# yanqinJiang/Animate3D

Measured on NVIDIA H100. Metric: MV-VDM denoise-steps/sec @ 4view x 16frame x 256^2, higher is better.
Workload: dtype fp16

## Files before the change

### animate3d_b200/csrc/a3d_attn.cu

```cuda
#include <stdlib.h>

#include "a3d_common.cuh"
#include "a3d_host.cuh"
#include "a3d_wgmma.cuh"

namespace a3d {

struct AttnDev {
  int q_tiles, kv_tiles;
  int rows_q, rows_k;
  int heads;
  int q_t1, q_box1, q_box2, q_e1, q_e3;
  int k_t1, k_box1, k_box2, k_e3, kv_div, kv_i3_zero;
  uint32_t q_box_bytes, k_box_bytes;
  float scale_log2;
  __half* out;
  int64_t os1, os2, os3, os4;
  int accumulate;
  float out_scale;
  unsigned long long* dbg;
};

constexpr float kRescaleLog2 = 8.0f;
constexpr int kAttnThreads = 288;

template <int D>
struct AttnCfg {
  static constexpr int kDqk = (D + 15) / 16 * 16;
  static constexpr int kDv = (D + 1 + 15) / 16 * 16;
  static constexpr int kQB = (kDqk + 63) / 64;
  static constexpr int kVB = (kDv + 63) / 64;
  static constexpr int kStages = (D == 160) ? 3 : 4;
  static constexpr int kQBox = 128 * 128;
  static constexpr int kKVBox = 64 * 128;
  static constexpr int kSmemQ = kQB * kQBox;
  static constexpr int kSmemK = kStages * kQB * kKVBox;
  static constexpr int kSmemV = kStages * kVB * kKVBox;
  static constexpr int kSmemBytes = kSmemQ + kSmemK + kSmemV + 1024 + 256;
  static constexpr int kMinBlocks = (kSmemBytes <= 113 * 1024) ? 2 : 1;
  static_assert(kSmemBytes <= 227 * 1024, "shared memory budget");
};

template <int N>
__device__ __forceinline__ void wgmma_pv(float (&o)[N / 2], const uint32_t (&a)[4], uint64_t bdesc, uint32_t acc) {
  if constexpr (N == 48) wgmma_rs_n48<1>(o, a, bdesc, acc);
  else if constexpr (N == 96) wgmma_rs_n96<1>(o, a, bdesc, acc);
  else wgmma_rs_n176<1>(o, a, bdesc, acc);
}

template <int D>
__global__ void __launch_bounds__(kAttnThreads, AttnCfg<D>::kMinBlocks)
attn_tc_kernel(const AttnDev p, const __grid_constant__ CUtensorMap mapQ, const __grid_constant__ CUtensorMap mapK,
               const __grid_constant__ CUtensorMap mapV) {
  using Cfg = AttnCfg<D>;
  constexpr int S = Cfg::kStages;
  extern __shared__ uint8_t smem_raw[];
  uint8_t* smem = reinterpret_cast<uint8_t*>((reinterpret_cast<uintptr_t>(smem_raw) + 1023) & ~uintptr_t(1023));
  uint8_t* sQ = smem;
  uint8_t* sK = sQ + Cfg::kSmemQ;
  uint8_t* sV = sK + Cfg::kSmemK;
  uint64_t* bars = reinterpret_cast<uint64_t*>(sV + Cfg::kSmemV);
  uint64_t* q_full = bars;
  uint64_t* k_full = bars + 1;
  uint64_t* v_full = k_full + S;
  uint64_t* kv_empty = v_full + S;

  const int warp = threadIdx.x >> 5;
  const int lane = threadIdx.x & 31;
  const int qt = blockIdx.x;
  const int head = blockIdx.y;
  const int qb = blockIdx.z;
  const int n = p.kv_tiles;
  const int rows_tile = p.k_box1 * p.k_box2;

  if (p.rows_q < 128 || rows_tile < 64) {
    uint4* z = reinterpret_cast<uint4*>(sQ);
    const int n16 = (Cfg::kSmemQ + Cfg::kSmemK + Cfg::kSmemV) / 16;
    for (int i = threadIdx.x; i < n16; i += blockDim.x) z[i] = make_uint4(0, 0, 0, 0);
    fence_proxy_async_smem();
  }
  if (warp == 8 && lane == 0) {
    tma_prefetch_desc(&mapQ);
    tma_prefetch_desc(&mapK);
    tma_prefetch_desc(&mapV);
    mbar_init(q_full, 1);
    for (int i = 0; i < S; ++i) {
      mbar_init(&k_full[i], 1);
      mbar_init(&v_full[i], 1);
      mbar_init(&kv_empty[i], 8);
    }
    mbar_fence_init();
  }
  __syncthreads();

  const int q_i1 = (qt % p.q_t1) * p.q_box1;
  const int q_i2 = (qt / p.q_t1) * p.q_box2;
  const int q_i3 = qb % p.q_e3;
  const int q_i4 = qb / p.q_e3;

  if (warp == 8) {
    if (lane == 0) {
      const int kb = qb / p.kv_div;
      const int k_i3 = p.kv_i3_zero ? 0 : (kb % p.k_e3);
      const int k_i4 = kb / p.k_e3;
      mbar_expect_tx(q_full, p.q_box_bytes * Cfg::kQB);
#pragma unroll
      for (int b = 0; b < Cfg::kQB; ++b)
        tma_load_5d(sQ + b * Cfg::kQBox, &mapQ, q_full, head * Cfg::kDqk + b * 64, q_i1, q_i2, q_i3, q_i4);
      for (int j = 0; j < n; ++j) {
        const int st = j % S;
        const int k_i1 = (j % p.k_t1) * p.k_box1, k_i2 = (j / p.k_t1) * p.k_box2;
        mbar_wait(&kv_empty[st], ((j / S) & 1) ^ 1);
        mbar_expect_tx(&k_full[st], p.k_box_bytes * Cfg::kQB);
#pragma unroll
        for (int b = 0; b < Cfg::kQB; ++b)
          tma_load_5d(sK + (st * Cfg::kQB + b) * Cfg::kKVBox, &mapK, &k_full[st], head * Cfg::kDqk + b * 64, k_i1, k_i2, k_i3,
                      k_i4);
        mbar_expect_tx(&v_full[st], p.k_box_bytes * Cfg::kVB);
#pragma unroll
        for (int b = 0; b < Cfg::kVB; ++b)
          tma_load_5d(sV + (st * Cfg::kVB + b) * Cfg::kKVBox, &mapV, &v_full[st], head * Cfg::kDv + b * 64, k_i1, k_i2, k_i3,
                      k_i4);
      }
    }
    return;
  }

  const int wg = warp >> 2;
  const int g = lane >> 2, t = lane & 3;
  float s[32];
  float o[Cfg::kDv / 2];
#pragma unroll
  for (int i = 0; i < Cfg::kDv / 2; ++i) o[i] = 0.f;
  float m_lo = -INFINITY, m_hi = -INFINITY;
  const uint32_t q0 = smem_u32(sQ + wg * (64 * 128));
  mbar_wait(q_full, 0);
  for (int j = 0; j < n; ++j) {
    const int st = j % S;
    const uint32_t ph = (j / S) & 1;
    mbar_wait(&k_full[st], ph);
    wgmma_fence();
#pragma unroll
    for (int kk = 0; kk < Cfg::kDqk / 16; ++kk) {
      const uint64_t qd = make_smem_desc_sw128(q0 + (kk / 4) * Cfg::kQBox + (kk % 4) * 32, 16, 1024);
      const uint64_t kd = make_smem_desc_sw128(smem_u32(sK + (st * Cfg::kQB + kk / 4) * Cfg::kKVBox) + (kk % 4) * 32, 16, 1024);
      wgmma_ss_n64<0>(s, qd, kd, kk ? 1u : 0u);
    }
    wgmma_commit();
    wgmma_wait<0>();
    reg_fence(s);
    const int valid = (j == n - 1) ? p.rows_k : rows_tile;
    float mx_lo = -INFINITY, mx_hi = -INFINITY;
#pragma unroll
    for (int jj = 0; jj < 8; ++jj) {
#pragma unroll
      for (int e = 0; e < 2; ++e) {
        if (8 * jj + 2 * t + e >= valid) { s[4 * jj + e] = -INFINITY; s[4 * jj + 2 + e] = -INFINITY; }
        mx_lo = fmaxf(mx_lo, s[4 * jj + e]);
        mx_hi = fmaxf(mx_hi, s[4 * jj + 2 + e]);
      }
    }
#pragma unroll
    for (int x = 1; x <= 2; x <<= 1) {
      mx_lo = fmaxf(mx_lo, __shfl_xor_sync(0xffffffffu, mx_lo, x));
      mx_hi = fmaxf(mx_hi, __shfl_xor_sync(0xffffffffu, mx_hi, x));
    }
    const float mn_lo = fmaxf(m_lo, mx_lo * p.scale_log2), mn_hi = fmaxf(m_hi, mx_hi * p.scale_log2);
    if (j == 0) {
      m_lo = mn_lo; m_hi = mn_hi;
    } else if (__any_sync(0xffffffffu, mn_lo - m_lo > kRescaleLog2 || mn_hi - m_hi > kRescaleLog2)) {
      if (p.dbg && lane == 0) atomicAdd(p.dbg, 1ull);
      const float a_lo = ex2_approx(m_lo - mn_lo), a_hi = ex2_approx(m_hi - mn_hi);
#pragma unroll
      for (int c = 0; c < Cfg::kDv / 8; ++c) {
        o[4 * c] *= a_lo; o[4 * c + 1] *= a_lo; o[4 * c + 2] *= a_hi; o[4 * c + 3] *= a_hi;
      }
      m_lo = mn_lo; m_hi = mn_hi;
    }
    uint32_t pa[4][4];
#pragma unroll
    for (int kk = 0; kk < 4; ++kk) {
#pragma unroll
      for (int h = 0; h < 2; ++h) {
        const float* sb = s + 4 * (2 * kk + h);
        pa[kk][2 * h] = pack_f16x2(ex2_approx(fmaf(sb[0], p.scale_log2, -m_lo)), ex2_approx(fmaf(sb[1], p.scale_log2, -m_lo)));
        pa[kk][2 * h + 1] = pack_f16x2(ex2_approx(fmaf(sb[2], p.scale_log2, -m_hi)), ex2_approx(fmaf(sb[3], p.scale_log2, -m_hi)));
      }
    }
    mbar_wait(&v_full[st], ph);
    wgmma_fence();
#pragma unroll
    for (int kk = 0; kk < 4; ++kk) {
      const uint64_t vd = make_smem_desc_sw128(smem_u32(sV + st * Cfg::kVB * Cfg::kKVBox) + kk * 2048, Cfg::kKVBox, 1024);
      wgmma_pv<Cfg::kDv>(o, pa[kk], vd, 1u);
    }
    wgmma_commit();
    wgmma_wait<0>();
    reg_fence(o);
    __syncwarp();
    if (lane == 0) mbar_arrive(&kv_empty[st]);
  }
  const float l_lo = __shfl_sync(0xffffffffu, o[4 * (D / 8)], lane & ~3);
  const float l_hi = __shfl_sync(0xffffffffu, o[4 * (D / 8) + 2], lane & ~3);
#pragma unroll
  for (int h = 0; h < 2; ++h) {
    const int r = wg * 64 + (warp & 3) * 16 + g + 8 * h;
    const int i1 = q_i1 + r % p.q_box1;
    if (r >= p.rows_q || i1 >= p.q_e1) continue;
    const float inv = p.out_scale / (h ? l_hi : l_lo);
    const int i2 = q_i2 + r / p.q_box1;
    __half* orow = p.out + (int64_t)i1 * p.os1 + (int64_t)i2 * p.os2 + (int64_t)q_i3 * p.os3 + (int64_t)q_i4 * p.os4 +
                   head * D + 2 * t;
#pragma unroll
    for (int c = 0; c < D / 8; ++c) {
      float v0 = o[4 * c + 2 * h] * inv, v1 = o[4 * c + 2 * h + 1] * inv;
      if (p.accumulate) {
        const float2 f = __half22float2(*reinterpret_cast<const __half2*>(orow + 8 * c));
        v0 += f.x; v1 += f.y;
      }
      *reinterpret_cast<uint32_t*>(orow + 8 * c) = pack_f16x2(v0, v1);
    }
  }
}

struct ViewDev {
  const __half* base;
  int64_t s1, s2, s3, s4;
  int e1, e2, e3, e4;
};

__global__ void attn_simt_kernel(ViewDev q, ViewDev k, ViewDev v, __half* out, int64_t os1, int64_t os2, int64_t os3,
                                 int64_t os4, int heads, int d, int dqk, int dv, float scale, int kv_div, int kv_i3_zero,
                                 int accumulate, float out_scale) {
  const int Lq = q.e1 * q.e2, Lk = k.e1 * k.e2;
  const int64_t total = (int64_t)q.e3 * q.e4 * heads * Lq;
  const int64_t idx = (int64_t)blockIdx.x * blockDim.x + threadIdx.x;
  if (idx >= total) return;
  const int l = (int)(idx % Lq);
  const int h = (int)((idx / Lq) % heads);
  const int qb = (int)(idx / ((int64_t)Lq * heads));
  const int kb = qb / kv_div;
  const __half* qp = q.base + (int64_t)(l % q.e1) * q.s1 + (int64_t)(l / q.e1) * q.s2 + (int64_t)(qb % q.e3) * q.s3 +
                     (int64_t)(qb / q.e3) * q.s4 + h * dqk;
  const int64_t koff = (int64_t)(kv_i3_zero ? 0 : kb % k.e3) * k.s3 + (int64_t)(kb / k.e3) * k.s4;
  const int64_t voff = (int64_t)(kv_i3_zero ? 0 : kb % v.e3) * v.s3 + (int64_t)(kb / v.e3) * v.s4;
  float m = -INFINITY;
  for (int j = 0; j < Lk; ++j) {
    const __half* kp = k.base + koff + (int64_t)(j % k.e1) * k.s1 + (int64_t)(j / k.e1) * k.s2 + h * dqk;
    float s = 0.f;
    for (int c = 0; c < d; ++c) s += __half2float(qp[c]) * __half2float(kp[c]);
    m = fmaxf(m, s * scale);
  }
  float acc[160];
  for (int c = 0; c < d; ++c) acc[c] = 0.f;
  float sum = 0.f;
  for (int j = 0; j < Lk; ++j) {
    const __half* kp = k.base + koff + (int64_t)(j % k.e1) * k.s1 + (int64_t)(j / k.e1) * k.s2 + h * dqk;
    const __half* vp = v.base + voff + (int64_t)(j % v.e1) * v.s1 + (int64_t)(j / v.e1) * v.s2 + h * dv;
    float s = 0.f;
    for (int c = 0; c < d; ++c) s += __half2float(qp[c]) * __half2float(kp[c]);
    const float pj = expf(s * scale - m);
    sum += pj;
    for (int c = 0; c < d; ++c) acc[c] += pj * __half2float(vp[c]);
  }
  __half* op = out + (int64_t)(l % q.e1) * os1 + (int64_t)(l / q.e1) * os2 + (int64_t)(qb % q.e3) * os3 +
               (int64_t)(qb / q.e3) * os4 + h * d;
  for (int c = 0; c < d; ++c) {
    float o = out_scale * acc[c] / sum;
    if (accumulate) o += __half2float(op[c]);
    op[c] = __float2half_rn(o);
  }
}

constexpr int kFewKeysMax = 8;

template <int D>
__global__ void __launch_bounds__(256)
attn_fewkeys_kernel(ViewDev q, ViewDev k, ViewDev v, __half* out, int64_t os1, int64_t os2, int64_t os3, int64_t os4, int heads,
                    int dqk, int dv, float scale_log2, int kv_div, int kv_i3_zero, int accumulate, float out_scale) {
  constexpr int d = D;
  const int Lq = q.e1 * q.e2, Lk = k.e1 * k.e2;
  const int64_t total = (int64_t)q.e3 * q.e4 * Lq * heads;
  const int64_t idx = (int64_t)blockIdx.x * blockDim.x + threadIdx.x;
// ... 401 lines not shown
```

### animate3d_b200/csrc/a3d_gemm.cu

```cuda
#include <type_traits>

#include "a3d_common.cuh"
#include "a3d_host.cuh"
#include "a3d_wgmma.cuh"

namespace a3d {

struct GemmDev {
  int64_t M, N, K;
  int num_k_blocks;
  int tiles_m, tiles_n;
  int a_mode;
  int cpb;
  int conv_s;
  int tpi;
  int boh;
  int bimg;
  int tpr;
  int conv_pad;
  const float* bias;
  const float* rowbias;
  int64_t rb_ld, rb_div, rb_mod;
  float acc_scale;
  const __half* R1; int64_t ldr1; float r1_scale;
  const __half* R2; int64_t ldr2;
  void* C; int64_t ldc;
  int geglu, out_f32;
  int64_t perm_a, perm_b;
  long long* trace;
};

__device__ __forceinline__ float gelu_erf(float x) {
  float t;
  asm("rcp.approx.ftz.f32 %0, %1;" : "=f"(t) : "f"(fmaf(0.3275911f * 0.70710678118654752f, fabsf(x), 1.0f)));
  float poly = fmaf(1.061405429f, t, -1.453152027f);
  poly = fmaf(poly, t, 1.421413741f);
  poly = fmaf(poly, t, -0.284496736f);
  poly = fmaf(poly, t, 0.254829592f);
  const float xs = x * 0.84932180028801904f;
  const float e = ex2_approx(-xs * xs);
  const float erf_abs = fmaf(-(poly * t), e, 1.0f);
  const float h = 0.5f * x;
  return fmaf(fabsf(h), erf_abs, h);
}

__device__ __forceinline__ int64_t perm_row(int64_t m, int64_t a, int64_t b) {
  if (a == 0) return m;
  const int64_t ab = a * b;
  return (m / ab) * ab + (m % b) * a + (m / b) % a;
}

constexpr int kBM = 128;
constexpr int kBK = 64;
constexpr int kGemmThreads = 288;

template <int BN>
struct GemmCfg {
  static constexpr int kABytes = kBM * kBK * 2;
  static constexpr int kBBytes = BN * kBK * 2;
  static constexpr int kStageBytes = kABytes + kBBytes;
  static constexpr int kStages = (227 * 1024 - 1024 - 256) / kStageBytes > 6 ? 6 : (227 * 1024 - 1024 - 256) / kStageBytes;
  static constexpr int kSmemBytes = kStages * kStageBytes + 1024  + 256 ;
  static_assert(kSmemBytes <= 227 * 1024, "shared memory budget");
};

template <int BN>
__device__ __forceinline__ void wgmma_tile(float (&d)[BN / 2], uint64_t adesc, uint64_t bdesc, uint32_t acc) {
  if constexpr (BN == 256) wgmma_ss_n256<0>(d, adesc, bdesc, acc);
  else if constexpr (BN == 160) wgmma_ss_n160<0>(d, adesc, bdesc, acc);
  else wgmma_ss_n128<0>(d, adesc, bdesc, acc);
}

enum { kEpiPlain = 0, kEpiRes = 1, kEpiGeglu = 2, kEpiF32 = 3, kEpiGelu = 4 };

template <int BN, int EPI>
struct EpiChunk {
  static constexpr int G = BN == 256 ? 1 + (EPI == kEpiGeglu) : 2;
  static constexpr bool kAhead = BN != 256;
  float bias[G][2];
  float rb[2][G][2];
  uint32_t r1[2][G], r2[2][G];
};

template <int EPI, int G>
__device__ __forceinline__ constexpr int epi_group(int c, int s) {
  if constexpr (EPI != kEpiGeglu) {
    return c * G + s;
  } else {
    const int o = c * (G / 2) + s % (G / 2);
    return (o / 4) * 8 + o % 4 + (s >= G / 2 ? 4 : 0);
  }
}

__device__ __forceinline__ void prefetch_l2(const void* a) { asm volatile("prefetch.global.L2 [%0];" ::"l"(a)); }

template <int BN, int EPI>
__global__ void __launch_bounds__(kGemmThreads, 1)
gemm_tc_kernel(const GemmDev p, const __grid_constant__ CUtensorMap mapA, const __grid_constant__ CUtensorMap mapB) {
  static_assert(EPI != kEpiGeglu || BN % 64 == 0, "GEGLU pairs a value with its gate inside 64-column blocks");
  static_assert((BN / 8) % EpiChunk<BN, EPI>::G == 0, "the tile's column groups split into whole chunks");
  using Cfg = GemmCfg<BN>;
  constexpr int kStages = Cfg::kStages;
  extern __shared__ uint8_t smem_raw[];
  uint8_t* smem = reinterpret_cast<uint8_t*>((reinterpret_cast<uintptr_t>(smem_raw) + 1023) & ~uintptr_t(1023));
  uint8_t* smem_a = smem;
  uint8_t* smem_b = smem + kStages * Cfg::kABytes;
  uint64_t* full_bar = reinterpret_cast<uint64_t*>(smem + kStages * Cfg::kStageBytes);
  uint64_t* empty_bar = full_bar + kStages;

  const int warp = threadIdx.x >> 5;
  const int lane = threadIdx.x & 31;
  const int num_tiles = p.tiles_m * p.tiles_n;

  if (warp == 8 && lane == 0) {
    tma_prefetch_desc(&mapA);
    tma_prefetch_desc(&mapB);
    for (int i = 0; i < kStages; ++i) {
      mbar_init(&full_bar[i], 1);
      mbar_init(&empty_bar[i], 8);
    }
    mbar_fence_init();
  }
  __syncthreads();

  if (warp == 8) {
    if (lane == 0) {
      int stage = 0;
      uint32_t phase = 0;
      for (int tile = blockIdx.x; tile < num_tiles; tile += gridDim.x) {
        const int mt = tile / p.tiles_n, nt = tile % p.tiles_n;
        int img0 = 0, oh0 = 0, ow0 = 0;
        if (p.a_mode == A3D_A_CONV3) {
          if (p.tpr > 1) { img0 = mt / p.tpi; oh0 = (mt % p.tpi) / p.tpr; ow0 = ((mt % p.tpi) % p.tpr) * kBM; }
          else if (p.tpi > 0) { img0 = mt / p.tpi; oh0 = (mt % p.tpi) * p.boh; }
          else { img0 = mt * p.bimg; oh0 = 0; }
        }
        for (int kb = 0; kb < p.num_k_blocks; ++kb) {
          mbar_wait(&empty_bar[stage], phase ^ 1);
          mbar_expect_tx(&full_bar[stage], Cfg::kStageBytes);
          if (p.a_mode == A3D_A_CONV3) {
            const int tap = kb / p.cpb, c0 = (kb % p.cpb) * kBK;
            const int ky = tap / 3, kx = tap % 3;
            tma_load_5d(smem_a + stage * Cfg::kABytes, &mapA, &full_bar[stage], c0, ow0 * p.conv_s + kx - p.conv_pad,
                        oh0 * p.conv_s + ky - p.conv_pad, img0, 0);
          } else {
            tma_load_5d(smem_a + stage * Cfg::kABytes, &mapA, &full_bar[stage], kb * kBK, mt * kBM, 0, 0, 0);
          }
          tma_load_5d(smem_b + stage * Cfg::kBBytes, &mapB, &full_bar[stage], kb * kBK, nt * BN, 0, 0, 0);
          if (++stage == kStages) { stage = 0; phase ^= 1; }
        }
      }
    }
    return;
  }

  const int wg = warp >> 2;
  const int g = lane >> 2, t = lane & 3;
  int stage = 0;
  uint32_t phase = 0;
  int tcount = 0;
  float acc[BN / 2];
  for (int tile = blockIdx.x; tile < num_tiles; tile += gridDim.x, ++tcount) {
    const int mt = tile / p.tiles_n, nt = tile % p.tiles_n;
    const bool tr = p.trace && blockIdx.x == 0 && threadIdx.x == 0 && tcount < 60;
    if (tr) p.trace[tcount * 16 + 0] = clock64();
    const int64_t col_base = (int64_t)nt * BN + 2 * t;
    int64_t row[2], orow[2];
#pragma unroll
    for (int h = 0; h < 2; ++h) {
      row[h] = (int64_t)mt * kBM + wg * 64 + (warp & 3) * 16 + g + 8 * h;
      orow[h] = (EPI == kEpiRes) ? perm_row(row[h], p.perm_a, p.perm_b) : row[h];
    }
    int prev_stage = -1;
    for (int kb = 0; kb < p.num_k_blocks; ++kb) {
      if constexpr (EPI == kEpiRes) {
        if (kb == (p.num_k_blocks > 2 ? p.num_k_blocks - 2 : 0)) {
          const int64_t ncols = p.N - (int64_t)nt * BN < BN ? p.N - (int64_t)nt * BN : BN;
          auto fetch = [&](const __half* a, bool ok) {
            const uintptr_t e = reinterpret_cast<uintptr_t>(a + ncols), l0 = reinterpret_cast<uintptr_t>(a) & ~uintptr_t(127);
#pragma unroll
            for (int i = 0; i < (2 * BN / 128 + 4) / 4; ++i) {
              const uintptr_t l = l0 + 128 * (t + 4 * i);
              if (ok && l < e) prefetch_l2(reinterpret_cast<const void*>(l));
            }
          };
#pragma unroll
          for (int h = 0; h < 2; ++h) {
            fetch(p.R1 + row[h] * p.ldr1 + (int64_t)nt * BN, p.R1 && row[h] < p.M);
            fetch(p.R2 + orow[h] * p.ldr2 + (int64_t)nt * BN, p.R2 && row[h] < p.M);
          }
        }
      }
      mbar_wait(&full_bar[stage], phase);
      const uint32_t a0 = smem_u32(smem_a + stage * Cfg::kABytes + wg * (64 * 128));
      const uint32_t b0 = smem_u32(smem_b + stage * Cfg::kBBytes);
      wgmma_fence();
#pragma unroll
      for (int k = 0; k < kBK / 16; ++k)
        wgmma_tile<BN>(acc, make_smem_desc_sw128(a0 + 32 * k, 16, 1024), make_smem_desc_sw128(b0 + 32 * k, 16, 1024),
                       (kb | k) ? 1u : 0u);
      wgmma_commit();
      wgmma_wait<1>();
      if (prev_stage >= 0 && lane == 0) mbar_arrive(&empty_bar[prev_stage]);
      prev_stage = stage;
      if (++stage == kStages) { stage = 0; phase ^= 1; }
    }

    using Chunk = EpiChunk<BN, EPI>;
    constexpr int G = Chunk::G;
    constexpr int kChunks = BN / 8 / G;
    const float* rb[2];
#pragma unroll
    for (int h = 0; h < 2; ++h) rb[h] = p.rowbias ? p.rowbias + ((row[h] / p.rb_div) % p.rb_mod) * p.rb_ld : nullptr;
    Chunk op;
    auto load_chunk = [&](int c) {
#pragma unroll
      for (int s = 0; s < G; ++s) {
        const int64_t n = col_base + 8 * epi_group<EPI, G>(c, s);
        const bool col_ok = n < p.N;
        op.bias[s][0] = (p.bias && col_ok) ? p.bias[n] : 0.f;
        op.bias[s][1] = (p.bias && col_ok) ? p.bias[n + 1] : 0.f;
#pragma unroll
        for (int h = 0; h < 2; ++h) {
          const bool ok = col_ok && row[h] < p.M;
          op.rb[h][s][0] = (rb[h] && ok) ? rb[h][n] : 0.f;
          op.rb[h][s][1] = (rb[h] && ok) ? rb[h][n + 1] : 0.f;
          if constexpr (EPI == kEpiRes) {
            op.r1[h][s] = (p.R1 && ok) ? *reinterpret_cast<const uint32_t*>(p.R1 + row[h] * p.ldr1 + n) : 0u;
            op.r2[h][s] = (p.R2 && ok) ? *reinterpret_cast<const uint32_t*>(p.R2 + orow[h] * p.ldr2 + n) : 0u;
          }
        }
      }
    };
    auto finish = [&](float v, int h, int s, int e) {
      if (p.bias) v += op.bias[s][e];
      if (rb[h]) v += op.rb[h][s][e];
      return v * p.acc_scale;
    };
    auto half2_float2 = [](uint32_t u) { return __half22float2(*reinterpret_cast<const __half2*>(&u)); };

    if constexpr (Chunk::kAhead) load_chunk(0);
    wgmma_wait<0>();
    reg_fence(acc);
    if (lane == 0) mbar_arrive(&empty_bar[prev_stage]);
    if (tr) p.trace[tcount * 16 + 1] = clock64();

#pragma unroll
    for (int c = 0; c < kChunks; ++c) {
      if constexpr (!Chunk::kAhead) load_chunk(c);
      if constexpr (EPI == kEpiGeglu) {
        uint32_t out[2][G / 2];
#pragma unroll
        for (int h = 0; h < 2; ++h)
#pragma unroll
          for (int s = 0; s < G / 2; ++s) {
            const int ju = epi_group<EPI, G>(c, s), jg = epi_group<EPI, G>(c, s + G / 2);
            const float u0 = finish(acc[4 * ju + 2 * h], h, s, 0), u1 = finish(acc[4 * ju + 2 * h + 1], h, s, 1);
            const float g0 = finish(acc[4 * jg + 2 * h], h, s + G / 2, 0), g1 = finish(acc[4 * jg + 2 * h + 1], h, s + G / 2, 1);
            out[h][s] = pack_f16x2(u0 * gelu_erf(g0), u1 * gelu_erf(g1));
          }
        if (Chunk::kAhead && c + 1 < kChunks) load_chunk(c + 1);
#pragma unroll
        for (int h = 0; h < 2; ++h) {
          if (row[h] >= p.M) continue;
          __half* crow = reinterpret_cast<__half*>(p.C) + row[h] * p.ldc;
#pragma unroll
          for (int s = 0; s < G / 2; ++s) {
            if (col_base + 8 * epi_group<EPI, G>(c, s) >= p.N) continue;
            const int o = c * (G / 2) + s;
            *reinterpret_cast<uint32_t*>(crow + (int64_t)nt * (BN / 2) + 8 * o + 2 * t) = out[h][s];
          }
        }
      } else if constexpr (EPI == kEpiF32) {
        float out[2][G][2];
#pragma unroll
        for (int h = 0; h < 2; ++h)
#pragma unroll
          for (int s = 0; s < G; ++s)
#pragma unroll
            for (int e = 0; e < 2; ++e) out[h][s][e] = finish(acc[4 * (c * G + s) + 2 * h + e], h, s, e);
        if (Chunk::kAhead && c + 1 < kChunks) load_chunk(c + 1);
#pragma unroll
        for (int h = 0; h < 2; ++h) {
          if (row[h] >= p.M) continue;
          float* crow = reinterpret_cast<float*>(p.C) + row[h] * p.ldc;
#pragma unroll
          for (int s = 0; s < G; ++s) {
            const int64_t n = col_base + 8 * (c * G + s);
            if (n >= p.N) continue;
            crow[n] = out[h][s][0];
            crow[n + 1] = out[h][s][1];
// ... 11 lines not shown
              v0 = gelu_erf(v0); v1 = gelu_erf(v1);
            }
            if constexpr (EPI == kEpiRes) {
              if (p.R1) {
                const float2 f = half2_float2(op.r1[h][s]);
                v0 += p.r1_scale * f.x; v1 += p.r1_scale * f.y;
              }
              if (p.R2) {
                const float2 f = half2_float2(op.r2[h][s]);
                v0 += f.x; v1 += f.y;
              }
            }
            out[h][s] = pack_f16x2(v0, v1);
          }
        if (Chunk::kAhead && c + 1 < kChunks) load_chunk(c + 1);
#pragma unroll
        for (int h = 0; h < 2; ++h) {
          if (row[h] >= p.M) continue;
          __half* crow = reinterpret_cast<__half*>(p.C) + orow[h] * p.ldc;
#pragma unroll
          for (int s = 0; s < G; ++s) {
            const int64_t n = col_base + 8 * (c * G + s);
            if (n >= p.N) continue;
            *reinterpret_cast<uint32_t*>(crow + n) = out[h][s];
          }
        }
      }
    }
    if (tr) p.trace[tcount * 16 + 2] = clock64();
  }
}

struct SimtConv { int n, h, w, c, s, oh, ow, pad; };

__global__ void gemm_simt_kernel(const GemmDev p, const __half* __restrict__ A, int64_t lda, const __half* __restrict__ B,
                                 SimtConv cv) {
  const int64_t n_out = p.geglu == 1 ? p.N / 2 : p.N;
  const int64_t idx = (int64_t)blockIdx.x * blockDim.x + threadIdx.x;
  if (idx >= p.M * n_out) return;
  const int64_t m = idx / n_out;
  const int64_t j = idx % n_out;
  auto dot = [&](int64_t n) {
    float acc = 0.f;
    const __half* b = B + n * p.K;
    if (p.a_mode == A3D_A_PLAIN) {
      const __half* a = A + m * lda;
      for (int64_t k = 0; k < p.K; ++k) acc += __half2float(a[k]) * __half2float(b[k]);
    } else {
      const int img = (int)(m / (cv.oh * cv.ow));
      const int oy = (int)((m / cv.ow) % cv.oh), ox = (int)(m % cv.ow);
      for (int tap = 0; tap < 9; ++tap) {
        const int iy = oy * cv.s + tap / 3 - cv.pad, ix = ox * cv.s + tap % 3 - cv.pad;
        if (iy < 0 || iy >= cv.h || ix < 0 || ix >= cv.w) continue;
        const __half* a = A + (((int64_t)img * cv.h + iy) * cv.w + ix) * cv.c;
        const __half* bb = b + (int64_t)tap * cv.c;
        for (int c = 0; c < cv.c; ++c) acc += __half2float(a[c]) * __half2float(bb[c]);
      }
    }
    return acc;
  };
  const int64_t orow = perm_row(m, p.perm_a, p.perm_b);
  const float* rb = p.rowbias ? p.rowbias + ((m / p.rb_div) % p.rb_mod) * p.rb_ld : nullptr;
  auto finish = [&](int64_t n) {
    float v = dot(n);
    if (p.bias) v += p.bias[n];
    if (rb) v += rb[n];
    return v * p.acc_scale;
  };
  if (p.geglu == 1) {
    const int64_t blk = j / 32, e = j % 32;
    const int64_t nu = blk * 64 + e, ng = nu + 32;
    const float u = finish(nu), g = finish(ng);
    reinterpret_cast<__half*>(p.C)[orow * p.ldc + j] = __float2half_rn(u * gelu_erf(g));
    return;
  }
  float v = finish(j);
  if (p.geglu == 2) v = gelu_erf(v);
  if (p.R1) v += p.r1_scale * __half2float(p.R1[m * p.ldr1 + j]);
  if (p.R2) v += __half2float(p.R2[orow * p.ldr2 + j]);
  if (p.out_f32) reinterpret_cast<float*>(p.C)[orow * p.ldc + j] = v;
  else reinterpret_cast<__half*>(p.C)[orow * p.ldc + j] = __float2half_rn(v);
}

template <int BN, int EPI>
static int launch_tc_epi(const GemmDev& dev, const CUtensorMap* mapA, const CUtensorMap* mapB, cudaStream_t st) {
  using Cfg = GemmCfg<BN>;
  static bool attr_set = false;
  if (!attr_set) {
    A3D_CUDA_CHECK(cudaFuncSetAttribute(gemm_tc_kernel<BN, EPI>, cudaFuncAttributeMaxDynamicSharedMemorySize, Cfg::kSmemBytes));
    attr_set = true;
  }
  const int tiles = dev.tiles_m * dev.tiles_n;
  const int grid = tiles < sm_count() ? tiles : sm_count();
  gemm_tc_kernel<BN, EPI><<<grid, kGemmThreads, Cfg::kSmemBytes, st>>>(dev, *mapA, *mapB);
  A3D_LAUNCH_CHECK();
  return A3D_OK;
}

template <int BN>
static int launch_tc(const GemmDev& dev, const CUtensorMap* mapA, const CUtensorMap* mapB, cudaStream_t st) {
  if (dev.out_f32) return launch_tc_epi<BN, kEpiF32>(dev, mapA, mapB, st);
  if (dev.geglu == 1) {
    if constexpr (BN % 64 == 0) return launch_tc_epi<BN, kEpiGeglu>(dev, mapA, mapB, st);
    else return fail(A3D_EINVAL, "a3d_gemm: GEGLU needs a 128- or 256-column tile");
  }
  if (dev.geglu == 2) return launch_tc_epi<BN, kEpiGelu>(dev, mapA, mapB, st);
  if (dev.R1 || dev.R2 || dev.perm_a) return launch_tc_epi<BN, kEpiRes>(dev, mapA, mapB, st);
  return launch_tc_epi<BN, kEpiPlain>(dev, mapA, mapB, st);
}

static long long* g_gemm_trace = nullptr;

}

extern "C" int a3d_debug_set_gemm_trace(void* device_buffer_1024_int64) {
  a3d::g_gemm_trace = reinterpret_cast<long long*>(device_buffer_1024_int64);
  return A3D_OK;
}

extern "C" int a3d_gemm(const a3d_gemm_args* a, void* stream) {
  using namespace a3d;
  cudaStream_t st = reinterpret_cast<cudaStream_t>(stream);
  if (!a || !a->A || !a->B || !a->C) return fail(A3D_EINVAL, "a3d_gemm: null operand");
  if (a->M <= 0 || a->N <= 0 || a->K <= 0) return fail(A3D_EINVAL, "a3d_gemm: empty problem M=%lld N=%lld K=%lld",
                                                        (long long)a->M, (long long)a->N, (long long)a->K);
  GemmDev d;
  memset(&d, 0, sizeof(d));
  d.M = a->M; d.N = a->N; d.K = a->K;
  d.a_mode = a->a_mode;
  d.bias = a->bias; d.rowbias = a->rowbias; d.rb_ld = a->rb_ld;
  d.rb_div = a->rb_div > 0 ? a->rb_div : 1; d.rb_mod = a->rb_mod > 0 ? a->rb_mod : (int64_t)1 << 40;
  d.acc_scale = a->acc_scale;
  d.R1 = reinterpret_cast<const __half*>(a->R1); d.ldr1 = a->ldr1; d.r1_scale = a->r1_scale;
  d.R2 = reinterpret_cast<const __half*>(a->R2); d.ldr2 = a->ldr2;
  d.C = a->C; d.ldc = a->ldc; d.geglu = a->geglu; d.out_f32 = a->out_f32;
  d.perm_a = a->perm_a; d.perm_b = a->perm_b;
  d.trace = g_gemm_trace;
  if (a->geglu < 0 || a->geglu > 2) return fail(A3D_EINVAL, "a3d_gemm: geglu must be 0 (none), 1 (GEGLU) or 2 (GELU)");
  const bool geglu = a->geglu == 1;
  if (geglu && (a->out_f32 || a->R1 || a->R2 || a->perm_a || (a->N % 128)))
    return fail(A3D_EINVAL, "a3d_gemm: GEGLU epilogue takes bias / row-bias only, fp16 output, N %% 128 == 0");
  if (a->geglu == 2 && (a->out_f32 || a->R1 || a->R2 || a->perm_a))
    return fail(A3D_EINVAL, "a3d_gemm: GELU epilogue takes bias / row-bias only, fp16 output");
  if (a->out_f32 && (a->R1 || a->R2 || a->perm_a))
    return fail(A3D_EINVAL, "a3d_gemm: fp32 output supports bias / row-bias only");

  SimtConv cv{0, 0, 0, 0, 1, 0, 0};
  if (a->a_mode == A3D_A_CONV3) {
    const int s = a->conv_stride;
    if (s != 1 && s != 2) return fail(A3D_EINVAL, "a3d_gemm: conv stride must be 1 or 2");
    if (a->conv_h % s || a->conv_w % s) return fail(A3D_EINVAL, "a3d_gemm: conv H/W must be multiples of the stride");
    cv = SimtConv{a->conv_n, a->conv_h, a->conv_w, a->conv_c, s, a->conv_h / s, a->conv_w / s, a->conv_nopad_lo ? 0 : 1};
    if (a->K != 9LL * a->conv_c || a->M != (int64_t)cv.n * cv.oh * cv.ow)
      return fail(A3D_EINVAL, "a3d_gemm: conv geometry does not match M/K");
    d.conv_s = s;
  } else if (a->a_mode != A3D_A_PLAIN) {
    return fail(A3D_EINVAL, "a3d_gemm: unknown a_mode %d", a->a_mode);
  }

  bool tc_ok = (a->K % kBK == 0) && (a->N % (geglu ? 16 : 8) == 0) && ((reinterpret_cast<uintptr_t>(a->A) & 15) == 0) &&
               ((reinterpret_cast<uintptr_t>(a->B) & 15) == 0) && (a->ldc % 16 == 0) &&
               ((reinterpret_cast<uintptr_t>(a->C) & 31) == 0);
  if (a->a_mode == A3D_A_PLAIN) tc_ok = tc_ok && (a->lda % 8 == 0) && a->lda >= a->K;
  int boh = 0, bimg = 1, tpi = 0, tpr = 1;
  if (a->a_mode == A3D_A_CONV3) {
    tc_ok = tc_ok && (cv.c % kBK == 0);
    const int opix = cv.oh * cv.ow;
    if (cv.ow > kBM) {
      tc_ok = tc_ok && (cv.ow % kBM == 0);
      boh = 1; tpr = cv.ow / kBM; tpi = cv.oh * tpr; bimg = 1;
    } else if (opix >= kBM) {
      tc_ok = tc_ok && (opix % kBM == 0) && (kBM % cv.ow == 0);
      boh = kBM / cv.ow; tpi = opix / kBM; bimg = 1;
    } else {
      tc_ok = tc_ok && (kBM % opix == 0);
      boh = cv.oh; tpi = 0; bimg = kBM / (opix > 0 ? opix : 1);
    }
    tc_ok = tc_ok && (tpr > 1 ? kBM : cv.ow) * cv.s <= 256 && boh * cv.s <= 256;
  }
  if (a->R1) tc_ok = tc_ok && (a->ldr1 % 16 == 0) && ((reinterpret_cast<uintptr_t>(a->R1) & 31) == 0);
  if (a->R2) tc_ok = tc_ok && (a->ldr2 % 16 == 0) && ((reinterpret_cast<uintptr_t>(a->R2) & 31) == 0);
  int impl = a->impl;
  if (impl == A3D_GEMM_AUTO) impl = tc_ok ? A3D_GEMM_TCGEN05 : A3D_GEMM_SIMT;
  if (impl == A3D_GEMM_TCGEN05 && !tc_ok)
    return fail(A3D_EINVAL, "a3d_gemm: shape/alignment not supported by the tensor-core path (M=%lld N=%lld K=%lld)",
                (long long)a->M, (long long)a->N, (long long)a->K);

  if (impl == A3D_GEMM_SIMT) {
    const int64_t n_out = geglu ? a->N / 2 : a->N;
    const int64_t total = a->M * n_out;
    const int threads = 128;
    const int64_t blocks = (total + threads - 1) / threads;
    gemm_simt_kernel<<<(unsigned)blocks, threads, 0, st>>>(d, reinterpret_cast<const __half*>(a->A), a->lda,
                                                           reinterpret_cast<const __half*>(a->B), cv);
    A3D_LAUNCH_CHECK();
    return A3D_OK;
  }

  int BN;
  if (geglu) BN = (a->N % 256 == 0) ? 256 : 128;
  else if (a->N % 256 == 0) BN = 256;
  else if (a->K <= 640 && a->N > 512 && (256 * ((a->N + 255) / 256) - a->N) * 8 <= a->N) {
    BN = 256;
  } else if (a->N % 160 == 0) BN = 160;
  else BN = 128;
  {
    static int force = -1;
    if (force < 0) { const char* e = getenv("A3D_GEMM_BN"); force = e ? atoi(e) : 0; }
    if (!geglu && (force == 128 || force == 160 || force == 256)) BN = force;
  }
  if (geglu && a->N % BN) return fail(A3D_EINVAL, "a3d_gemm: GEGLU needs N %% 128 == 0");
  d.num_k_blocks = (int)(a->K / kBK);
  d.tiles_m = (int)((a->M + kBM - 1) / kBM);
  d.tiles_n = (int)((a->N + BN - 1) / BN);
  d.cpb = a->a_mode == A3D_A_CONV3 ? cv.c / kBK : 0;
  d.tpi = tpi; d.boh = boh; d.bimg = bimg; d.tpr = tpr; d.conv_pad = cv.pad;
  const CUtensorMap *mapA = nullptr, *mapB = nullptr;
  {
    MapKey kb;
    const uint64_t dims[5] = {(uint64_t)a->K, (uint64_t)a->N, 1, 1, 1};
    const uint64_t str[4] = {(uint64_t)a->K, (uint64_t)a->K * a->N, (uint64_t)a->K * a->N, (uint64_t)a->K * a->N};
    const uint32_t box[5] = {kBK, (uint32_t)BN, 1, 1, 1};
    kb = make_key(a->B, dims, str, box);
    if (int r = get_tensor_map(kb, &mapB)) return r;
  }
  if (a->a_mode == A3D_A_PLAIN) {
    const uint64_t dims[5] = {(uint64_t)a->K, (uint64_t)a->M, 1, 1, 1};
    const uint64_t str[4] = {(uint64_t)a->lda, (uint64_t)a->lda * a->M, (uint64_t)a->lda * a->M, (uint64_t)a->lda * a->M};
    const uint32_t box[5] = {kBK, kBM, 1, 1, 1};
    MapKey ka = make_key(a->A, dims, str, box);
    if (int r = get_tensor_map(ka, &mapA)) return r;
  } else {
    const uint64_t img = (uint64_t)cv.h * cv.w * cv.c;
    const uint64_t dims[5] = {(uint64_t)cv.c, (uint64_t)cv.w, (uint64_t)cv.h, (uint64_t)cv.n, 1};
    const uint64_t str[4] = {(uint64_t)cv.c, (uint64_t)cv.w * cv.c, img, img * cv.n};
    const uint32_t box[5] = {kBK, (uint32_t)((tpr > 1 ? kBM : cv.ow) * cv.s), (uint32_t)(boh * cv.s), (uint32_t)bimg, 1};
    MapKey ka = make_key(a->A, dims, str, box);
    ka.estr[1] = cv.s; ka.estr[2] = cv.s;
    if (int r = get_tensor_map(ka, &mapA)) return r;
  }
  switch (BN) {
    case 256: return launch_tc<256>(d, mapA, mapB, st);
    case 160: return launch_tc<160>(d, mapA, mapB, st);
    default: return launch_tc<128>(d, mapA, mapB, st);
  }
}
```

Measured before the change: 5.657.

## Overlap next QK^T wgmma with current PV wgmma in attention consumer loop

Restructures the consumer warpgroup loop so the S=QK^T wgmma for tile j is issued before the PV wgmma for tile j-1, then waits with wgmma_wait<1> so the softmax of tile j runs while PV is still in flight. The goal is to hide tensor-core latency behind exp/max work. For D=40 the old serial order is kept. It also precomputes the smem descriptors once, skips masking for full tiles, and replaces launch_bounds with a __maxnreg__ cap. The extra live registers (P fragments plus scores plus O) may cause spills, especially at large head dims.

```diff
diff --git a/animate3d_b200/csrc/a3d_attn.cu b/animate3d_b200/csrc/a3d_attn.cu
--- a/animate3d_b200/csrc/a3d_attn.cu
+++ b/animate3d_b200/csrc/a3d_attn.cu
@@ -38,6 +38,8 @@
   static constexpr int kSmemV = kStages * kVB * kKVBox;
   static constexpr int kSmemBytes = kSmemQ + kSmemK + kSmemV + 1024 + 256;
   static constexpr int kMinBlocks = (kSmemBytes <= 113 * 1024) ? 2 : 1;
+  static constexpr bool kPipelined = D != 40;
+  static constexpr int kMaxRegs = 65536 / (kMinBlocks * kAttnThreads) / 8 * 8;
   static_assert(kSmemBytes <= 227 * 1024, "shared memory budget");
 };
 
@@ -49,7 +51,7 @@
 }
 
 template <int D>
-__global__ void __launch_bounds__(kAttnThreads, AttnCfg<D>::kMinBlocks)
+__global__ void __maxnreg__(AttnCfg<D>::kMaxRegs)
 attn_tc_kernel(const AttnDev p, const __grid_constant__ CUtensorMap mapQ, const __grid_constant__ CUtensorMap mapK,
                const __grid_constant__ CUtensorMap mapV) {
   using Cfg = AttnCfg<D>;
@@ -128,34 +130,47 @@
 
   const int wg = warp >> 2;
   const int g = lane >> 2, t = lane & 3;
+  const float sl2 = p.scale_log2;
   float s[32];
   float o[Cfg::kDv / 2];
+  uint32_t pa[4][4];
 #pragma unroll
   for (int i = 0; i < Cfg::kDv / 2; ++i) o[i] = 0.f;
   float m_lo = -INFINITY, m_hi = -INFINITY;
-  const uint32_t q0 = smem_u32(sQ + wg * (64 * 128));
-  mbar_wait(q_full, 0);
-  for (int j = 0; j < n; ++j) {
-    const int st = j % S;
-    const uint32_t ph = (j / S) & 1;
-    mbar_wait(&k_full[st], ph);
+  const uint64_t qdesc = make_smem_desc_sw128(smem_u32(sQ + wg * (64 * 128)), 16, 1024);
+  const uint64_t kdesc = make_smem_desc_sw128(smem_u32(sK), 16, 1024);
+  const uint64_t vdesc = make_smem_desc_sw128(smem_u32(sV), Cfg::kKVBox, 1024);
+
+  auto issue_s = [&](int st) {
+    const uint64_t kst = kdesc + (uint32_t)(st * (Cfg::kQB * Cfg::kKVBox / 16));
     wgmma_fence();
 #pragma unroll
-    for (int kk = 0; kk < Cfg::kDqk / 16; ++kk) {
-      const uint64_t qd = make_smem_desc_sw128(q0 + (kk / 4) * Cfg::kQBox + (kk % 4) * 32, 16, 1024);
-      const uint64_t kd = make_smem_desc_sw128(smem_u32(sK + (st * Cfg::kQB + kk / 4) * Cfg::kKVBox) + (kk % 4) * 32, 16, 1024);
-      wgmma_ss_n64<0>(s, qd, kd, kk ? 1u : 0u);
-    }
+    for (int kk = 0; kk < Cfg::kDqk / 16; ++kk)
+      wgmma_ss_n64<0>(s, qdesc + ((kk / 4) * Cfg::kQBox + (kk % 4) * 32) / 16, kst + ((kk / 4) * Cfg::kKVBox + (kk % 4) * 32) / 16,
+                      kk ? 1u : 0u);
     wgmma_commit();
-    wgmma_wait<0>();
-    reg_fence(s);
-    const int valid = (j == n - 1) ? p.rows_k : rows_tile;
-    float mx_lo = -INFINITY, mx_hi = -INFINITY;
+  };
+  auto issue_pv = [&](int st) {
+    const uint64_t vst = vdesc + (uint32_t)(st * (Cfg::kVB * Cfg::kKVBox / 16));
+    wgmma_fence();
+#pragma unroll
+    for (int kk = 0; kk < 4; ++kk) wgmma_pv<Cfg::kDv>(o, pa[kk], vst + kk * 2048 / 16, 1u);
+    wgmma_commit();
+  };
+  auto row_max = [&](int valid, float& mx_lo, float& mx_hi) {
+    if (valid < 64) {
+#pragma unroll
+      for (int jj = 0; jj < 8; ++jj) {
+#pragma unroll
+        for (int e = 0; e < 2; ++e)
+          if (8 * jj + 2 * t + e >= valid) { s[4 * jj + e] = -INFINITY; s[4 * jj + 2 + e] = -INFINITY; }
+      }
+    }
+    mx_lo = -INFINITY; mx_hi = -INFINITY;
 #pragma unroll
     for (int jj = 0; jj < 8; ++jj) {
 #pragma unroll
       for (int e = 0; e < 2; ++e) {
-        if (8 * jj + 2 * t + e >= valid) { s[4 * jj + e] = -INFINITY; s[4 * jj + 2 + e] = -INFINITY; }
         mx_lo = fmaxf(mx_lo, s[4 * jj + e]);
         mx_hi = fmaxf(mx_hi, s[4 * jj + 2 + e]);
       }
@@ -165,40 +180,101 @@
       mx_lo = fmaxf(mx_lo, __shfl_xor_sync(0xffffffffu, mx_lo, x));
       mx_hi = fmaxf(mx_hi, __shfl_xor_sync(0xffffffffu, mx_hi, x));
     }
-    const float mn_lo = fmaxf(m_lo, mx_lo * p.scale_log2), mn_hi = fmaxf(m_hi, mx_hi * p.scale_log2);
-    if (j == 0) {
-      m_lo = mn_lo; m_hi = mn_hi;
-    } else if (__any_sync(0xffffffffu, mn_lo - m_lo > kRescaleLog2 || mn_hi - m_hi > kRescaleLog2)) {
-      if (p.dbg && lane == 0) atomicAdd(p.dbg, 1ull);
-      const float a_lo = ex2_approx(m_lo - mn_lo), a_hi = ex2_approx(m_hi - mn_hi);
-#pragma unroll
-      for (int c = 0; c < Cfg::kDv / 8; ++c) {
-        o[4 * c] *= a_lo; o[4 * c + 1] *= a_lo; o[4 * c + 2] *= a_hi; o[4 * c + 3] *= a_hi;
-      }
-      m_lo = mn_lo; m_hi = mn_hi;
-    }
-    uint32_t pa[4][4];
+  };
+  auto exp_scores = [&]() {
+#pragma unroll
+    for (int i = 0; i < 32; i += 4) {
+      s[i] = ex2_approx(fmaf(s[i], sl2, -m_lo)); s[i + 1] = ex2_approx(fmaf(s[i + 1], sl2, -m_lo));
+      s[i + 2] = ex2_approx(fmaf(s[i + 2], sl2, -m_hi)); s[i + 3] = ex2_approx(fmaf(s[i + 3], sl2, -m_hi));
+    }
+  };
+  auto pack_p = [&]() {
 #pragma unroll
     for (int kk = 0; kk < 4; ++kk) {
 #pragma unroll
       for (int h = 0; h < 2; ++h) {
         const float* sb = s + 4 * (2 * kk + h);
-        pa[kk][2 * h] = pack_f16x2(ex2_approx(fmaf(sb[0], p.scale_log2, -m_lo)), ex2_approx(fmaf(sb[1], p.scale_log2, -m_lo)));
-        pa[kk][2 * h + 1] = pack_f16x2(ex2_approx(fmaf(sb[2], p.scale_log2, -m_hi)), ex2_approx(fmaf(sb[3], p.scale_log2, -m_hi)));
-      }
-    }
-    mbar_wait(&v_full[st], ph);
-    wgmma_fence();
-#pragma unroll
-    for (int kk = 0; kk < 4; ++kk) {
-      const uint64_t vd = make_smem_desc_sw128(smem_u32(sV + st * Cfg::kVB * Cfg::kKVBox) + kk * 2048, Cfg::kKVBox, 1024);
-      wgmma_pv<Cfg::kDv>(o, pa[kk], vd, 1u);
-    }
-    wgmma_commit();
+        pa[kk][2 * h] = pack_f16x2(sb[0], sb[1]);
+        pa[kk][2 * h + 1] = pack_f16x2(sb[2], sb[3]);
+      }
+    }
+  };
+
+  mbar_wait(q_full, 0);
+  mbar_wait(&k_full[0], 0);
+  issue_s(0);
+  wgmma_wait<0>();
+  reg_fence(s);
+  {
+    float mx_lo, mx_hi;
+    row_max(n == 1 ? p.rows_k : rows_tile, mx_lo, mx_hi);
+    m_lo = fmaxf(m_lo, mx_lo * sl2); m_hi = fmaxf(m_hi, mx_hi * sl2);
+  }
+  exp_scores();
+  pack_p();
+  if constexpr (!Cfg::kPipelined) {
+    mbar_wait(&v_full[0], 0);
+    issue_pv(0);
     wgmma_wait<0>();
     reg_fence(o);
     __syncwarp();
-    if (lane == 0) mbar_arrive(&kv_empty[st]);
+    if (lane == 0) mbar_arrive(&kv_empty[0]);
+  }
+  int st = 0;
+  uint32_t ph = 0;
+  for (int j = 1; j < n; ++j) {
+    const int pst = st;
+    const uint32_t pph = ph;
+    if (++st == S) { st = 0; ph ^= 1; }
+    mbar_wait(&k_full[st], ph);
+    issue_s(st);
+    if constexpr (Cfg::kPipelined) {
+      mbar_wait(&v_full[pst], pph);
+      issue_pv(pst);
+      wgmma_wait<1>();
+    } else {
+      wgmma_wait<0>();
+    }
+    reg_fence(s);
+    float mx_lo, mx_hi;
+    row_max(j == n - 1 ? p.rows_k : rows_tile, mx_lo, mx_hi);
+    const float mn_lo = fmaxf(m_lo, mx_lo * sl2), mn_hi = fmaxf(m_hi, mx_hi * sl2);
+    const bool rescale = __any_sync(0xffffffffu, mn_lo - m_lo > kRescaleLog2 || mn_hi - m_hi > kRescaleLog2);
+    float a_lo = 1.f, a_hi = 1.f;
+    if (rescale) {
+      a_lo = ex2_approx(m_lo - mn_lo); a_hi = ex2_approx(m_hi - mn_hi);
+      m_lo = mn_lo; m_hi = mn_hi;
+    }
+    exp_scores();
+    if (rescale && p.dbg && lane == 0) atomicAdd(p.dbg, 1ull);
+    if constexpr (Cfg::kPipelined) {
+      reg_fence(s);
+      wgmma_wait<0>();
+      reg_fence(o);
+      __syncwarp();
+      if (lane == 0) mbar_arrive(&kv_empty[pst]);
+    }
+    if (rescale) {
+#pragma unroll
+      for (int c = 0; c < Cfg::kDv / 8; ++c) {
+        o[4 * c] *= a_lo; o[4 * c + 1] *= a_lo; o[4 * c + 2] *= a_hi; o[4 * c + 3] *= a_hi;
+      }
+    }
+    pack_p();
+    if constexpr (!Cfg::kPipelined) {
+      mbar_wait(&v_full[st], ph);
+      issue_pv(st);
+      wgmma_wait<0>();
+      reg_fence(o);
+      __syncwarp();
+      if (lane == 0) mbar_arrive(&kv_empty[st]);
+    }
+  }
+  if constexpr (Cfg::kPipelined) {
+    mbar_wait(&v_full[st], ph);
+    issue_pv(st);
+    wgmma_wait<0>();
+    reg_fence(o);
   }
   const float l_lo = __shfl_sync(0xffffffffu, o[4 * (D / 8)], lane & ~3);
   const float l_hi = __shfl_sync(0xffffffffu, o[4 * (D / 8) + 2], lane & ~3);
```

Result: faster. 5.989, median of 6 (+5.9%).

## Add single-warpgroup 64-row GEMM variant with three CTAs per SM for small-K

Applied to the files above, without the earlier changes.

Templates the tensor-core GEMM on the number of consumer warpgroups. A new 64x128 tile configuration uses one consumer warpgroup and sizes shared memory for three resident CTAs per SM. It is selected when N is large and K is small, the aim being better latency hiding and wave balance for short-K GEMMs. The heuristic that padded N to 256-wide tiles is also dropped. The trade-off is fewer pipeline stages per CTA and smaller tiles with less operand reuse, and the conv tiling now depends on the chosen tile height.

```diff
diff --git a/animate3d_b200/csrc/a3d_gemm.cu b/animate3d_b200/csrc/a3d_gemm.cu
--- a/animate3d_b200/csrc/a3d_gemm.cu
+++ b/animate3d_b200/csrc/a3d_gemm.cu
@@ -50,18 +50,22 @@
   return (m / ab) * ab + (m % b) * a + (m / b) % a;
 }
 
-constexpr int kBM = 128;
 constexpr int kBK = 64;
-constexpr int kGemmThreads = 288;
-
-template <int BN>
+
+template <int BN, int kWG>
 struct GemmCfg {
+  static_assert(kWG == 1 || kWG == 2, "one or two consumer warpgroups");
+  static constexpr int kMinBlocks = kWG == 1 ? 3 : 1;
+  static constexpr int kBM = 64 * kWG;
+  static constexpr int kThreads = 32 * (4 * kWG + 1);
   static constexpr int kABytes = kBM * kBK * 2;
   static constexpr int kBBytes = BN * kBK * 2;
   static constexpr int kStageBytes = kABytes + kBBytes;
-  static constexpr int kStages = (227 * 1024 - 1024 - 256) / kStageBytes > 6 ? 6 : (227 * 1024 - 1024 - 256) / kStageBytes;
-  static constexpr int kSmemBytes = kStages * kStageBytes + 1024  + 256 ;
-  static_assert(kSmemBytes <= 227 * 1024, "shared memory budget");
+  static constexpr int kBudget = 228 * 1024 / kMinBlocks - 1024;
+  static constexpr int kFixed = 1024  + 256 ;
+  static constexpr int kStages = (kBudget - kFixed) / kStageBytes > 6 ? 6 : (kBudget - kFixed) / kStageBytes;
+  static constexpr int kSmemBytes = kStages * kStageBytes + kFixed;
+  static_assert(kStages >= 2, "shared memory budget");
 };
 
 template <int BN>
@@ -73,10 +77,10 @@
 
 enum { kEpiPlain = 0, kEpiRes = 1, kEpiGeglu = 2, kEpiF32 = 3, kEpiGelu = 4 };
 
-template <int BN, int EPI>
+template <int BN, int EPI, int kWG>
 struct EpiChunk {
   static constexpr int G = BN == 256 ? 1 + (EPI == kEpiGeglu) : 2;
-  static constexpr bool kAhead = BN != 256;
+  static constexpr bool kAhead = BN != 256 && !(kWG == 1 && EPI == kEpiRes);
   float bias[G][2];
   float rb[2][G][2];
   uint32_t r1[2][G], r2[2][G];
@@ -94,13 +98,15 @@
 
 __device__ __forceinline__ void prefetch_l2(const void* a) { asm volatile("prefetch.global.L2 [%0];" ::"l"(a)); }
 
-template <int BN, int EPI>
-__global__ void __launch_bounds__(kGemmThreads, 1)
+template <int BN, int EPI, int kWG>
+__global__ void __launch_bounds__(GemmCfg<BN, kWG>::kThreads, GemmCfg<BN, kWG>::kMinBlocks)
 gemm_tc_kernel(const GemmDev p, const __grid_constant__ CUtensorMap mapA, const __grid_constant__ CUtensorMap mapB) {
   static_assert(EPI != kEpiGeglu || BN % 64 == 0, "GEGLU pairs a value with its gate inside 64-column blocks");
-  static_assert((BN / 8) % EpiChunk<BN, EPI>::G == 0, "the tile's column groups split into whole chunks");
-  using Cfg = GemmCfg<BN>;
+  static_assert((BN / 8) % EpiChunk<BN, EPI, kWG>::G == 0, "the tile's column groups split into whole chunks");
+  using Cfg = GemmCfg<BN, kWG>;
   constexpr int kStages = Cfg::kStages;
+  constexpr int kBM = Cfg::kBM;
+  constexpr int kProducer = 4 * kWG;
   extern __shared__ uint8_t smem_raw[];
   uint8_t* smem = reinterpret_cast<uint8_t*>((reinterpret_cast<uintptr_t>(smem_raw) + 1023) & ~uintptr_t(1023));
   uint8_t* smem_a = smem;
@@ -112,18 +118,18 @@
   const int lane = threadIdx.x & 31;
   const int num_tiles = p.tiles_m * p.tiles_n;
 
-  if (warp == 8 && lane == 0) {
+  if (warp == kProducer && lane == 0) {
     tma_prefetch_desc(&mapA);
     tma_prefetch_desc(&mapB);
     for (int i = 0; i < kStages; ++i) {
       mbar_init(&full_bar[i], 1);
-      mbar_init(&empty_bar[i], 8);
+      mbar_init(&empty_bar[i], 4 * kWG);
     }
     mbar_fence_init();
   }
   __syncthreads();
 
-  if (warp == 8) {
+  if (warp == kProducer) {
     if (lane == 0) {
       int stage = 0;
       uint32_t phase = 0;
@@ -206,7 +212,7 @@
       if (++stage == kStages) { stage = 0; phase ^= 1; }
     }
 
-    using Chunk = EpiChunk<BN, EPI>;
+    using Chunk = EpiChunk<BN, EPI, kWG>;
     constexpr int G = Chunk::G;
     constexpr int kChunks = BN / 8 / G;
     const float* rb[2];
@@ -384,31 +390,33 @@
   else reinterpret_cast<__half*>(p.C)[orow * p.ldc + j] = __float2half_rn(v);
 }
 
-template <int BN, int EPI>
+template <int BN, int EPI, int kWG>
 static int launch_tc_epi(const GemmDev& dev, const CUtensorMap* mapA, const CUtensorMap* mapB, cudaStream_t st) {
-  using Cfg = GemmCfg<BN>;
+  using Cfg = GemmCfg<BN, kWG>;
+  auto kernel = gemm_tc_kernel<BN, EPI, kWG>;
   static bool attr_set = false;
   if (!attr_set) {
-    A3D_CUDA_CHECK(cudaFuncSetAttribute(gemm_tc_kernel<BN, EPI>, cudaFuncAttributeMaxDynamicSharedMemorySize, Cfg::kSmemBytes));
+    A3D_CUDA_CHECK(cudaFuncSetAttribute(kernel, cudaFuncAttributeMaxDynamicSharedMemorySize, Cfg::kSmemBytes));
     attr_set = true;
   }
   const int tiles = dev.tiles_m * dev.tiles_n;
-  const int grid = tiles < sm_count() ? tiles : sm_count();
-  gemm_tc_kernel<BN, EPI><<<grid, kGemmThreads, Cfg::kSmemBytes, st>>>(dev, *mapA, *mapB);
+  const int slots = Cfg::kMinBlocks * sm_count();
+  const int grid = tiles < slots ? tiles : slots;
+  kernel<<<grid, Cfg::kThreads, Cfg::kSmemBytes, st>>>(dev, *mapA, *mapB);
   A3D_LAUNCH_CHECK();
   return A3D_OK;
 }
 
-template <int BN>
+template <int BN, int kWG>
 static int launch_tc(const GemmDev& dev, const CUtensorMap* mapA, const CUtensorMap* mapB, cudaStream_t st) {
-  if (dev.out_f32) return launch_tc_epi<BN, kEpiF32>(dev, mapA, mapB, st);
+  if (dev.out_f32) return launch_tc_epi<BN, kEpiF32, kWG>(dev, mapA, mapB, st);
   if (dev.geglu == 1) {
-    if constexpr (BN % 64 == 0) return launch_tc_epi<BN, kEpiGeglu>(dev, mapA, mapB, st);
+    if constexpr (BN % 64 == 0) return launch_tc_epi<BN, kEpiGeglu, kWG>(dev, mapA, mapB, st);
     else return fail(A3D_EINVAL, "a3d_gemm: GEGLU needs a 128- or 256-column tile");
   }
-  if (dev.geglu == 2) return launch_tc_epi<BN, kEpiGelu>(dev, mapA, mapB, st);
-  if (dev.R1 || dev.R2 || dev.perm_a) return launch_tc_epi<BN, kEpiRes>(dev, mapA, mapB, st);
-  return launch_tc_epi<BN, kEpiPlain>(dev, mapA, mapB, st);
+  if (dev.geglu == 2) return launch_tc_epi<BN, kEpiGelu, kWG>(dev, mapA, mapB, st);
+  if (dev.R1 || dev.R2 || dev.perm_a) return launch_tc_epi<BN, kEpiRes, kWG>(dev, mapA, mapB, st);
+  return launch_tc_epi<BN, kEpiPlain, kWG>(dev, mapA, mapB, st);
 }
 
 static long long* g_gemm_trace = nullptr;
@@ -460,6 +468,9 @@
     return fail(A3D_EINVAL, "a3d_gemm: unknown a_mode %d", a->a_mode);
   }
 
+  const int wg = (a->N > 640 && a->K <= (geglu ? 320 : 640)) ? 1 : 2;
+  const int bm = 64 * wg;
+
   bool tc_ok = (a->K % kBK == 0) && (a->N % (geglu ? 16 : 8) == 0) && ((reinterpret_cast<uintptr_t>(a->A) & 15) == 0) &&
                ((reinterpret_cast<uintptr_t>(a->B) & 15) == 0) && (a->ldc % 16 == 0) &&
                ((reinterpret_cast<uintptr_t>(a->C) & 31) == 0);
@@ -468,17 +479,17 @@
   if (a->a_mode == A3D_A_CONV3) {
     tc_ok = tc_ok && (cv.c % kBK == 0);
     const int opix = cv.oh * cv.ow;
-    if (cv.ow > kBM) {
-      tc_ok = tc_ok && (cv.ow % kBM == 0);
-      boh = 1; tpr = cv.ow / kBM; tpi = cv.oh * tpr; bimg = 1;
-    } else if (opix >= kBM) {
-      tc_ok = tc_ok && (opix % kBM == 0) && (kBM % cv.ow == 0);
-      boh = kBM / cv.ow; tpi = opix / kBM; bimg = 1;
+    if (cv.ow > bm) {
+      tc_ok = tc_ok && (cv.ow % bm == 0);
+      boh = 1; tpr = cv.ow / bm; tpi = cv.oh * tpr; bimg = 1;
+    } else if (opix >= bm) {
+      tc_ok = tc_ok && (opix % bm == 0) && (bm % cv.ow == 0);
+      boh = bm / cv.ow; tpi = opix / bm; bimg = 1;
     } else {
-      tc_ok = tc_ok && (kBM % opix == 0);
-      boh = cv.oh; tpi = 0; bimg = kBM / (opix > 0 ? opix : 1);
-    }
-    tc_ok = tc_ok && (tpr > 1 ? kBM : cv.ow) * cv.s <= 256 && boh * cv.s <= 256;
+      tc_ok = tc_ok && (bm % opix == 0);
+      boh = cv.oh; tpi = 0; bimg = bm / (opix > 0 ? opix : 1);
+    }
+    tc_ok = tc_ok && (tpr > 1 ? bm : cv.ow) * cv.s <= 256 && boh * cv.s <= 256;
   }
   if (a->R1) tc_ok = tc_ok && (a->ldr1 % 16 == 0) && ((reinterpret_cast<uintptr_t>(a->R1) & 31) == 0);
   if (a->R2) tc_ok = tc_ok && (a->ldr2 % 16 == 0) && ((reinterpret_cast<uintptr_t>(a->R2) & 31) == 0);
@@ -500,20 +511,19 @@
   }
 
   int BN;
-  if (geglu) BN = (a->N % 256 == 0) ? 256 : 128;
+  if (wg == 1) BN = 128;
+  else if (geglu) BN = (a->N % 256 == 0) ? 256 : 128;
   else if (a->N % 256 == 0) BN = 256;
-  else if (a->K <= 640 && a->N > 512 && (256 * ((a->N + 255) / 256) - a->N) * 8 <= a->N) {
-    BN = 256;
-  } else if (a->N % 160 == 0) BN = 160;
+  else if (a->N % 160 == 0) BN = 160;
   else BN = 128;
-  {
+  if (wg == 2) {
     static int force = -1;
     if (force < 0) { const char* e = getenv("A3D_GEMM_BN"); force = e ? atoi(e) : 0; }
     if (!geglu && (force == 128 || force == 160 || force == 256)) BN = force;
   }
   if (geglu && a->N % BN) return fail(A3D_EINVAL, "a3d_gemm: GEGLU needs N %% 128 == 0");
   d.num_k_blocks = (int)(a->K / kBK);
-  d.tiles_m = (int)((a->M + kBM - 1) / kBM);
+  d.tiles_m = (int)((a->M + bm - 1) / bm);
   d.tiles_n = (int)((a->N + BN - 1) / BN);
   d.cpb = a->a_mode == A3D_A_CONV3 ? cv.c / kBK : 0;
   d.tpi = tpi; d.boh = boh; d.bimg = bimg; d.tpr = tpr; d.conv_pad = cv.pad;
@@ -529,21 +539,22 @@
   if (a->a_mode == A3D_A_PLAIN) {
     const uint64_t dims[5] = {(uint64_t)a->K, (uint64_t)a->M, 1, 1, 1};
     const uint64_t str[4] = {(uint64_t)a->lda, (uint64_t)a->lda * a->M, (uint64_t)a->lda * a->M, (uint64_t)a->lda * a->M};
-    const uint32_t box[5] = {kBK, kBM, 1, 1, 1};
+    const uint32_t box[5] = {kBK, (uint32_t)bm, 1, 1, 1};
     MapKey ka = make_key(a->A, dims, str, box);
     if (int r = get_tensor_map(ka, &mapA)) return r;
   } else {
     const uint64_t img = (uint64_t)cv.h * cv.w * cv.c;
     const uint64_t dims[5] = {(uint64_t)cv.c, (uint64_t)cv.w, (uint64_t)cv.h, (uint64_t)cv.n, 1};
     const uint64_t str[4] = {(uint64_t)cv.c, (uint64_t)cv.w * cv.c, img, img * cv.n};
-    const uint32_t box[5] = {kBK, (uint32_t)((tpr > 1 ? kBM : cv.ow) * cv.s), (uint32_t)(boh * cv.s), (uint32_t)bimg, 1};
+    const uint32_t box[5] = {kBK, (uint32_t)((tpr > 1 ? bm : cv.ow) * cv.s), (uint32_t)(boh * cv.s), (uint32_t)bimg, 1};
     MapKey ka = make_key(a->A, dims, str, box);
     ka.estr[1] = cv.s; ka.estr[2] = cv.s;
     if (int r = get_tensor_map(ka, &mapA)) return r;
   }
+  if (wg == 1) return launch_tc<128, 1>(d, mapA, mapB, st);
   switch (BN) {
-    case 256: return launch_tc<256>(d, mapA, mapB, st);
-    case 160: return launch_tc<160>(d, mapA, mapB, st);
-    default: return launch_tc<128>(d, mapA, mapB, st);
-  }
-}
+    case 256: return launch_tc<256, 2>(d, mapA, mapB, st);
+    case 160: return launch_tc<160, 2>(d, mapA, mapB, st);
+    default: return launch_tc<128, 2>(d, mapA, mapB, st);
+  }
+}
```

Result: faster. 5.736 before, 5.895 after, median of 6 (+2.8%).
